# s3prl/s3prl

Hardware: AMD Instinct MI355X
Metric: encoder-frames/sec (20 ms stride) HuBERT-base 32x10 s @16 kHz (higher is better)
Workload: dtype f32; 1 GPU; hubert_base random-init, 32x10 s @16 kHz per GPU, one UpstreamExpert.forward per step: all 13 hidden_states (fp32) written; utterances_per_gpu=32, global_batch=32, samples=160000, frames_per_utt=499, parallelism=dp1, lengths=equal, gather=none

## Files before the change

include/s3enc.h:

```cpp
#ifndef S3ENC_H
#define S3ENC_H

#include <stdint.h>

#ifdef __cplusplus
extern "C" {
#endif

#define S3ENC_VERSION 8
#define S3ENC_MAX_CONV 16
#define S3ENC_MAX_RES 4

typedef struct s3enc_encoder* s3enc_handle;

enum { S3ENC_HUBERT = 0, S3ENC_WAV2VEC2 = 1, S3ENC_WAVLM = 2,
       S3ENC_DISTILLER = 3,
       S3ENC_MULTIRES = 4,
       S3ENC_WAV2VEC = 5,
       S3ENC_CPC = 6,
       S3ENC_APC = 7,
       S3ENC_MOCKINGJAY = 8,
       S3ENC_DECOAR = 9,
       S3ENC_NPC = 10 };
enum { S3ENC_F32 = 0, S3ENC_BF16 = 1, S3ENC_F16 = 2,
// ... 203 lines not shown
                               int64_t recv_state_stride, int32_t n_states, int64_t bytes_per_state, void* const* ready_events,
                               void* stream);
int s3enc_comm_destroy(s3enc_comm c);

int s3enc_forward_padded(s3enc_handle h, const float* pcm, int64_t row_stride, const int64_t* lengths, int32_t B,
                         int64_t n_max, float* out, int64_t layer_stride, void* stream);

int s3enc_profile_enable(s3enc_handle h, int32_t on);
int s3enc_profile_reset(s3enc_handle h);
typedef struct s3enc_profile_entry {
    char name[48];
    int64_t launches;
    double ms;
    double flops;
    double bytes;
} s3enc_profile_entry;
int s3enc_profile_read(s3enc_handle h, s3enc_profile_entry* entries, int32_t max_entries, int32_t* n_entries);

int s3enc_debug_tap(s3enc_handle h, const char* name, float* host_out, int64_t max_elems, int64_t* n_elems);
int s3enc_debug_occupy_cus(int32_t workgroups, int32_t threads, double milliseconds, void* stream);
int s3enc_debug_clock_sample(uint64_t* out3_device, void* stream);
int s3enc_debug_gemm_schedule(int32_t M, int32_t N, int32_t batches, int32_t tm, int32_t tail, int32_t cus, int32_t* items4_host,
                              int64_t max_items, int64_t* n_items);

int s3enc_set_tuning(const char* key, int32_t value);
int s3enc_set_handle_tuning(s3enc_handle h, const char* key, int32_t value);


int s3enc_op_gemm(int32_t dtype, const void* A, int64_t lda, int64_t a_batch_stride, const void* W,
                  const float* bias, int32_t M, int32_t N, int32_t K, int32_t batches, int32_t act,
                  const float* residual, const int32_t* row_limit, float* out32, void* out16, int64_t ldo,
                  int64_t o_batch_stride, void* stream);

int s3enc_op_conv0(int32_t dtype, const float* const* wavs, const int64_t* lengths, int32_t B, int64_t n_max,
                   int32_t normalize, const float* w0, const float* bias, const float* gn_gamma, const float* gn_beta,
                   const float* ln_gamma, const float* ln_beta, int32_t C, int32_t stride, void* out, void* stream);
int s3enc_op_wavlm_gate(const float* x, const float* grep_w, const float* grep_b, const float* grep_a, int32_t B, int32_t T,
                        int32_t H, float* gate, void* stream);

int s3enc_op_layernorm(int32_t dtype, const float* x, const float* gamma, const float* beta, int32_t rows,
                       int32_t C, int32_t act, float* out32, void* out16, void* stream);

int s3enc_op_attention(int32_t dtype, const void* qkv, void* out, const int32_t* valid, int32_t B, int32_t T,
                       int32_t H, const float* bias_table, int32_t table_R, const float* gate, void* stream);

int s3enc_op_conformer_conv(const float* x, const float* taps, const float* shift, int32_t B, int32_t T, int32_t D, int32_t K,
                            float* out, void* stream);
int s3enc_op_relpos_attention(const float* qkv, float* out, const int32_t* valid, int32_t B, int32_t T, int32_t H, const float* P,
                              const float* qadd, void* stream);

int s3enc_op_gn1_apply(const float* x, const float* gamma, const float* beta, const float* res, float scale, int32_t log_compress,
                       int32_t B, int32_t rows, int32_t C, int32_t pad, int32_t pad_zero, float* dst, float* state, float* acc,
                       float acc_w, int32_t acc_norm, int32_t acc_init, void* stream);
int s3enc_op_argmax_gather(const float* scores, const float* table, int32_t shared, int64_t rows, int32_t G, int32_t V, int32_t Dv,
                           int64_t* ids, float* out, void* stream);

int s3enc_op_channelnorm_relu(const float* x, const float* gamma, const float* beta, int32_t B, int32_t rows, int32_t C,
                              int32_t pad, float* dst, float* state, void* stream);
int s3enc_op_rnn(int32_t cell, const float* pre, const float* w_hh_host, const float* b_hn, int32_t B, int32_t T, int32_t H,
                 int64_t ld_pre, float* out, int64_t ldo, void* stream);

int s3enc_op_rnn_len(int32_t cell, const float* pre, const float* w_hh_host, const float* b_hn, const int32_t* len_host,
                     const float* res, int64_t ld_res, int32_t B, int32_t T, int32_t H, int64_t ld_pre, float* out, int64_t ldo,
                     void* stream);

int s3enc_op_conv_taps(const float* x, const float* w_host, const float* bias, int32_t B, int32_t T, int32_t C, int32_t N, int32_t k,
// ... 48 lines not shown
```

s3prl_amd/_lib.py:

```python

from __future__ import annotations

import ctypes as C
import os

_HERE = os.path.dirname(os.path.abspath(__file__))
LIB_PATH = os.path.join(_HERE, "libs3enc.so")

S3ENC_MAX_CONV = 16
S3ENC_MAX_RES = 4
F32, BF16, F16, F32X3, F16X2 = 0, 1, 2, 3, 4
STATUS_NONFINITE, STATUS_PENDING = 1, 1 << 30
DTYPES = {"fp32": F32, "f32": F32, "float32": F32, "bf16": BF16, "bfloat16": BF16, "fp16": F16, "f16": F16,
          "float16": F16, "fp32x3": F32X3, "f32x3": F32X3, "bf16x3": F32X3,
          "fp16x2": F16X2, "f16x2": F16X2}
FAMILY = {"hubert": 0, "wav2vec2": 1, "wavlm": 2, "distiller": 3, "multires_hubert": 4, "wav2vec": 5, "cpc": 6, "apc": 7, "mockingjay": 8, "decoar": 9, "npc": 10}
CPC_NORM = {"layerNorm": 0, "instanceNorm": 1, "ID": 2, "batchNorm": 3}
CPC_AR = {"LSTM": 0, "GRU": 1, "RNN": 2, "transformer": 3, "no_ar": 4}
APC_WINDOW = {"povey": 0, "hamming": 1}
VQ_TYPE = {"none": 0, "gumbel": 1, "kmeans": 2}
SEL_HIDDEN, SEL_LAYER_OUT, SEL_FFN_OUT = 0, 1, 2
SELECTIONS = {None: SEL_HIDDEN, "hidden_states": SEL_HIDDEN, "fairseq_layers": SEL_LAYER_OUT,
              "fairseq_layers_before_residual": SEL_FFN_OUT}
ABI_VERSION = 8
# ... 103 lines not shown
    "s3enc_create_npc": (C.c_int, [C.POINTER(S3Config), C.POINTER(S3NpcConfig), C.POINTER(S3Tensor), _I32, _I32, C.POINTER(_VP)]),
    "s3enc_destroy": (C.c_int, [_VP]),
    "s3enc_num_frames": (C.c_int, [_VP, _I64, C.POINTER(_I32)]),
    "s3enc_num_output_frames": (C.c_int, [_VP, _I64, C.POINTER(_I32)]),
    "s3enc_downsample_rate": (C.c_int, [_VP, C.POINTER(_I32)]),
    "s3enc_valid_frames": (C.c_int, [_VP, _I64, _I64, C.POINTER(_I32)]),
    "s3enc_forward": (C.c_int, [_VP, C.POINTER(_VP), C.POINTER(_I64), _I32, _I64, _VP, _I64, _VP]),
    "s3enc_forward_status": (C.c_int, [_VP, _I32, C.POINTER(_I32)]),
    "s3enc_forward_ex": (C.c_int, [_VP, C.POINTER(_VP), C.POINTER(_I64), _I32, _I64, C.POINTER(S3ForwardOpts), _VP, _I64, _VP]),
    "s3enc_forward_aux": (C.c_int, [_VP, C.POINTER(_VP), C.POINTER(_I64), _I32, _I64, C.POINTER(S3ForwardOpts), _VP, _I64, _VP, _VP, _VP]),
    "s3enc_num_states": (C.c_int, [_VP, _I32, C.POINTER(_I32)]),
    "s3enc_forward_padded": (C.c_int, [_VP, _VP, _I64, C.POINTER(_I64), _I32, _I64, _VP, _I64, _VP]),
    "s3enc_set_layer_events": (C.c_int, [_VP, C.POINTER(_VP), _I32]),
    "s3enc_profile_enable": (C.c_int, [_VP, _I32]),
    "s3enc_profile_reset": (C.c_int, [_VP]),
    "s3enc_profile_read": (C.c_int, [_VP, C.POINTER(S3ProfileEntry), _I32, C.POINTER(_I32)]),
    "s3enc_debug_tap": (C.c_int, [_VP, C.c_char_p, C.POINTER(C.c_float), _I64, C.POINTER(_I64)]),
    "s3enc_comm_version": (C.c_int, [C.POINTER(_I32)]),
    "s3enc_comm_unique_id": (C.c_int, [_VP]),
    "s3enc_comm_init_rank": (C.c_int, [_VP, _I32, _I32, _I32, C.POINTER(_VP)]),
    "s3enc_comm_info": (C.c_int, [_VP, C.POINTER(_I32), C.POINTER(_I32)]),
    "s3enc_comm_allgather_states": (C.c_int, [_VP, _VP, _I64, _VP, _I64, _I32, _I64, C.POINTER(_VP), _VP]),
    "s3enc_comm_exchange_states": (C.c_int, [_VP, _I32, _VP, _I64, _VP, _I64, _I32, _I64, C.POINTER(_VP), _VP]),
    "s3enc_comm_destroy": (C.c_int, [_VP]),
    "s3enc_comm_init_local": (C.c_int, [_I32, _I32, _I32, C.POINTER(_VP)]),
    "s3enc_comm_copy_export": (C.c_int, [_VP, _VP, _I64, _VP]),
    "s3enc_comm_copy_attach": (C.c_int, [_VP, _VP]),
    "s3enc_comm_copy_status": (C.c_int, [_VP, C.POINTER(_I32)]),
    "s3enc_comm_copy_release": (C.c_int, [_VP, _VP]),
    "s3enc_set_handle_tuning": (C.c_int, [_VP, C.c_char_p, _I32]),
    "s3enc_set_tuning": (C.c_int, [C.c_char_p, _I32]),
    "s3enc_op_gemm": (C.c_int, [_I32, _VP, _I64, _I64, _VP, _VP, _I32, _I32, _I32, _I32, _I32, _VP, _VP, _VP, _VP,
                                _I64, _I64, _VP]),
    "s3enc_debug_occupy_cus": (C.c_int, [_I32, _I32, C.c_double, _VP]),
    "s3enc_debug_clock_sample": (C.c_int, [_VP, _VP]),
    "s3enc_debug_gemm_schedule": (C.c_int, [_I32, _I32, _I32, _I32, _I32, _I32, _VP, _I64, C.POINTER(_I64)]),
    "s3enc_op_layernorm": (C.c_int, [_I32, _VP, _VP, _VP, _I32, _I32, _I32, _VP, _VP, _VP]),
    "s3enc_op_attention": (C.c_int, [_I32, _VP, _VP, _VP, _I32, _I32, _I32, _VP, _I32, _VP, _VP]),
    "s3enc_op_conv0": (C.c_int, [_I32, C.POINTER(_VP), C.POINTER(_I64), _I32, _I64, _I32, _VP, _VP, _VP, _VP, _VP, _VP, _I32,
                                 _I32, _VP, _VP]),
    "s3enc_op_wavlm_gate": (C.c_int, [_VP, _VP, _VP, _VP, _I32, _I32, _I32, _VP, _VP]),
    "s3enc_op_conformer_conv": (C.c_int, [_VP, _VP, _VP, _I32, _I32, _I32, _I32, _VP, _VP]),
    "s3enc_op_gn1_apply": (C.c_int, [_VP, _VP, _VP, _VP, C.c_float, _I32, _I32, _I32, _I32, _I32, _I32, _VP, _VP, _VP, C.c_float,
                                     _I32, _I32, _VP]),
    "s3enc_op_channelnorm_relu": (C.c_int, [_VP, _VP, _VP, _I32, _I32, _I32, _I32, _VP, _VP, _VP]),
    "s3enc_op_rnn": (C.c_int, [_I32, _VP, _VP, _VP, _I32, _I32, _I32, _I64, _VP, _I64, _VP]),
    "s3enc_op_rnn_len": (C.c_int, [_I32, _VP, _VP, _VP, _VP, _VP, _I64, _I32, _I32, _I32, _I64, _VP, _I64, _VP]),
    "s3enc_op_lstm_bidir": (C.c_int, [_VP, _VP, _VP, _VP, _VP, _I32, _I32, _I32, _I64, _VP, _I64, _VP]),
    "s3enc_pack_lstm_bidir_whh": (C.c_int, [_VP, _I32, _VP]),
    "s3enc_op_conv_taps": (C.c_int, [_VP, _VP, _VP, _I32, _I32, _I32, _I32, _I32, _I32, _I32, _VP, _I64, _VP, _I32, _I64, _VP, _VP,
                                     _I32, _I32, _VP]),
    "s3enc_op_argmax_gather": (C.c_int, [_VP, _VP, _I32, _I64, _I32, _I32, _I32, _VP, _VP, _VP]),
    "s3enc_op_relpos_attention": (C.c_int, [_VP, _VP, _VP, _I32, _I32, _I32, _VP, _VP, _VP]),
    "s3enc_op_posconv": (C.c_int, [_I32, _VP, _VP, _VP, _I32, _I32, _I32, _I32, _I32, _VP, _VP]),
    "s3enc_weighted_sum": (C.c_int, [_VP, _I64, _I32, C.POINTER(C.c_float), _I32, _I64, _I32, _VP, _VP]),
    "s3enc_weighted_sum_backward_scratch": (_I64, [_I64, _I32]),
    "s3enc_weighted_sum_backward": (C.c_int, [_VP, _I64, _I32, _I32, _I64, _I32, _VP, _VP, _VP, _VP]),
    "s3enc_fbank_num_frames": (C.c_int, [C.POINTER(S3FbankConfig), _I64, C.POINTER(_I32)]),
    "s3enc_fbank_forward": (C.c_int, [C.POINTER(S3FbankConfig), _VP, C.POINTER(_I64), _I32, _VP, _I64, _I32, _VP]),
    "s3enc_fbank_forward_ex": (C.c_int, [C.POINTER(S3FbankConfig), _I32, _VP, C.POINTER(_I64), _I32, _VP, _I64, _I32, _VP]),
    "s3enc_logmel_frame_counts": (C.c_int, [C.POINTER(_I64), _I32, _I64, C.POINTER(_I32)]),
    "s3enc_logmel_forward": (C.c_int, [_VP, C.POINTER(_I64), _I32, _I64, _I32, C.c_float, _I32, C.POINTER(_I32), _VP, _I32, _VP]),
    "s3enc_op_layernorm_eps": (C.c_int, [_VP, _VP, _VP, C.c_float, _I64, _I32, _VP, _VP]),
    "s3enc_op_input_repr": (C.c_int, [_VP, _VP, _VP, _VP, _I32, _VP, _VP, C.c_float, _I64, _I32, _I32, _VP, _VP]),
}

# ... 187 lines not shown
```

s3prl_amd/csrc/engine.hip:

```cpp
#include "engine_internal.h"

namespace s3e {

thread_local std::string g_err;

long conv_len(const s3enc_config& c, long n, int upto ) {
    for (int i = 0; i < upto; ++i) n = n >= c.conv_kernel[i] ? (n - c.conv_kernel[i]) / c.conv_stride[i] + 1 : 0;
    return n;
}

int valid_frames(const s3enc_config& c, long length, long n_max) {
    const long T = conv_len(c, n_max, c.n_conv);
    if (T <= 0) return 0;
    long v;
    if (c.family == S3ENC_WAV2VEC2 || c.family == S3ENC_DISTILLER || c.family == S3ENC_WAV2VEC || c.family == S3ENC_APC || c.family == S3ENC_NPC) {
        v = conv_len(c, length, c.n_conv);
    } else {
        const long chunk = n_max / T;
        v = (length + chunk - 1) / chunk;
    }
    if (v > T) v = T;
    if (v < 0) v = 0;
    return (int)v;
}
// ... 328 lines not shown
            std::unique_ptr<MxImage> img(new MxImage());              \
            UP(upload_mx4_lo(*img, vec, N_, K_));                     \
            img->kind = KIND;                                         \
            e->mx_images[(buf).p] = std::move(img);                   \
        }                                                             \
    } while (0)

    if (e->x2 && !c.no_feature_layer_norm && c.n_conv >= 3) {
        bool ok = true;
        for (int i = 2; i < c.n_conv; ++i) ok = ok && x3_shape_ok(C, (long)c.conv_kernel[i] * C, (long)c.conv_stride[i] * C);
        if (ok) e->x2_conv_f32_from = 2;
        if (ok && tuning().fp16x2_conv1_f32 && x3_shape_ok(C, (long)c.conv_kernel[1] * C, (long)c.conv_stride[1] * C)) e->x2_conv_f32_from = 1;
    }
    e->conv.resize(c.n_conv);
    for (int i = 0; i < c.n_conv; ++i) {
        const std::string p = "feature_extractor.conv_layers." + std::to_string(i);
        const int cin = i == 0 ? 1 : C, k = c.conv_kernel[i];
        GET(p + ".0.weight", (long)C * cin * k, t);
        if (i == 0) {
            UP(upload_f32(e->conv[i].w, t));
        } else {
            tap_major(t, C, cin, k, t2);
            if (e->x2_conv_f32_from && i >= e->x2_conv_f32_from) {
                UP(upload_gemm_w(e->conv[i].w, t2, C, (long)k * cin, e->dtype, e->x2));
            } else {
                UPW(e->conv[i].w, t2, C, (long)k * cin, 1);
            }
            if (e->x3 || (e->x2_conv_f32_from && i >= e->x2_conv_f32_from)) UP(upload_x3(e->conv[i].w3, t2, C, (long)k * cin));
            if (e->dtype == F32 && !e->x3 && k == 3 && c.conv_stride[i] == 2) {
                std::vector<float> wp((size_t)C * cin);
                for (int co = 0; co < C; ++co)
                    for (int ci = 0; ci < cin; ++ci) wp[(size_t)co * cin + ci] = t2[(long)co * 3 * cin + ci] + t2[(long)co * 3 * cin + 2 * cin + ci];
                UP(upload_f32(e->conv[i].wp, wp));
            }
        }
        if (c.conv_bias) {
            GET(p + ".0.bias", C, t);
            UP(upload_f32(e->conv[i].bias, t));
            e->conv[i].has_bias = true;
        }
        if (c.extractor_layer_norm) {
            GET(p + ".2.1.weight", C, t);
            UP(upload_f32(e->conv[i].lng, t));
            GET(p + ".2.1.bias", C, t);
            UP(upload_f32(e->conv[i].lnb, t));
        } else if (i == 0) {
            GET(p + ".2.weight", C, t);
            UP(upload_f32(e->gn_g, t));
            GET(p + ".2.bias", C, t);
            UP(upload_f32(e->gn_b, t));
        }
    }
    if (!c.no_feature_layer_norm) {
        GET("layer_norm.weight", C, t);
        UP(upload_f32(e->fln_g, t));
        GET("layer_norm.bias", C, t);
        UP(upload_f32(e->fln_b, t));
    }
    GET("post_extract_proj.weight", (long)D * C, t);
    UP(upload_gemm_w(e->proj_w, t, D, C, e->dtype, e->x2));
    e->x2_proj_f32 = e->x2 && !c.no_feature_layer_norm && c.family != S3ENC_DISTILLER && x3_shape_ok(D, C, C);
    if (e->x3 || e->x2_proj_f32) UP(upload_x3(e->proj_w3, t, D, C));
    GET("post_extract_proj.bias", D, t);
    UP(upload_f32(e->proj_b, t));

    const bool conf = c.layer_type == 1;
// ... 630 lines not shown
    if (T < 1) return fail("s3enc_forward: input shorter than the receptive field of the conv stack");
    const long M = (long)B * T;
    MrPlan plan;
    if (mr) mr_plan(c, T, plan);
    for (const auto& bp : plan.blocks)
        if (bp.T < 1 || plan.T_out < 1) return fail("s3enc_forward: input too short for the coarsest resolution of the U-net");
    const long out_rows = mr ? (long)B * plan.T_out : M;
    if (check_out(out, fo, layer_stride, out_rows * D)) return 1;
    if (c.rel_pos && T > 6000) return fail("s3enc_forward: WavLM relative-position window limited to 6000 frames (120 s) per batch");
    if (conf && T > 100000) return fail("s3enc_forward: Conformer position tables are limited to 100000 frames (max_source_positions)");
    std::vector<int> valid(B);
    for (int b = 0; b < B; ++b) {
        valid[b] = valid_frames(c, lengths[b], n_max);
        if (valid[b] < 1) return fail("s3enc_forward: an utterance is too short to produce a valid frame");
    }
    std::vector<int> valid_blk;
    if (mr) {
        std::vector<int> v = valid;
        for (size_t bi = 1; bi < plan.blocks.size(); ++bi) {
            const MrBlockPlan& bp = plan.blocks[bi];
            const AdapterW& aw = e->mr_adapters[bp.adapter];
            const long up = aw.kind == 1 ? 1 : aw.up_rate, down = aw.kind == 2 ? 1 : aw.down_rate;
            for (int b = 0; b < B; ++b) {
                long nv = ((long)v[b] * up + down - 1) / down;
                v[b] = (int)std::min(nv, bp.T);
            }
            valid_blk.insert(valid_blk.end(), v.begin(), v.end());
            for (int b = 0; b < B; ++b) v[b] = (int)std::min<long>(v[b], bp.T_sum);
        }
    }
    DeviceGuard dg(e->device);
    if (!dg.ok) return fail("s3enc_forward: hipSetDevice failed");

    const size_t tbl_bytes = (size_t)B * (8 + 8 + 4) + valid_blk.size() * 4;
    const size_t part_elems = stats_partial_elems(B, n_max);
    {
        Bump sb(nullptr);
        sb.take(tbl_bytes);
        sb.take((size_t)B * sizeof(float2));
        sb.take((size_t)B * C * sizeof(float2));
        sb.take(part_elems * 8);
        HIP_TRY(e->small.ensure_on_stream(sb.off + 1024, st));
    }
    Bump sb(e->small.p);
    char* d_tbl = (char*)sb.take(tbl_bytes);
    float2* d_norm = (float2*)sb.take((size_t)B * sizeof(float2));
    float2* d_gn = (float2*)sb.take((size_t)B * C * sizeof(float2));
    double* d_part = (double*)sb.take(part_elems * 8);
    const float* const* d_ptrs = (const float* const*)d_tbl;
    const long* d_lens = (const long*)(d_tbl + (size_t)B * 8);
    const int* d_valid = (const int*)(d_tbl + (size_t)B * 16);

    char* hp;
    if (stage_begin(e, tbl_bytes, st, hp)) return 1;
    memcpy(hp, wav_ptrs_host, (size_t)B * 8);
    for (int b = 0; b < B; ++b) ((long*)(hp + (size_t)B * 8))[b] = (long)lengths[b];
    memcpy(hp + (size_t)B * 16, valid.data(), (size_t)B * 4);
    if (!valid_blk.empty()) memcpy(hp + (size_t)B * 20, valid_blk.data(), valid_blk.size() * 4);
    if (stage_commit(e, hp, d_tbl, tbl_bytes, st)) return 1;

    const bool lnmode = c.extractor_layer_norm != 0;
    const bool prel = c.layer_norm_first != 0;
    const bool gated = c.rel_pos && c.gru_rel_pos;
    const bool featln = !c.no_feature_layer_norm;
    const bool ffn_tap = fo.selection == S3ENC_SEL_FFN_OUT;
    const long HW = std::max<long>(F, (long)NH * D);
    void *actA, *actB, *tmp32, *feat32, *featT, *x32, *xpc, *xT, *qkv, *attn, *tmp1, *tmp2, *hbuf, *gate, *ffnbuf, *lnst, *cbuf, *pbuf;
    for (int pass = 0; pass < 2; ++pass) {
        Bump wb(pass ? e->ws.p : nullptr);
        actA = wb.take(std::max((size_t)B * L[0] * C * (e->x2_conv_f32_from == 1 ? 4 : es),
                                (e->x2_conv_f32_from && c.n_conv > 2) ? (size_t)B * L[2] * C * 4 : (size_t)0));
        actB = wb.take((size_t)B * L[1] * C * (e->x2_conv_f32_from ? 4 : es));
        tmp32 = lnmode ? wb.take((size_t)B * L[1] * C * 4) : nullptr;
        feat32 = featln ? wb.take((size_t)M * C * 4) : nullptr;
        featT = wb.take((size_t)M * C * (e->x2_proj_f32 ? 4 : es));
        x32 = wb.take((size_t)M * D * 4);
        xpc = wb.take((size_t)M * D * 4);
        xT = wb.take((size_t)M * D * es);
        qkv = wb.take((size_t)M * 3 * D * es);
        attn = wb.take((size_t)M * D * (e->x2_attn_f32 ? 4 : es));
        tmp1 = wb.take((size_t)M * D * 4);
        tmp2 = wb.take((size_t)M * D * 4);
        lnst = wb.take((size_t)M * sizeof(float2));
        hbuf = wb.take((size_t)M * HW * es);
        gate = gated ? wb.take((size_t)B * H * T * 4) : nullptr;
        ffnbuf = (ffn_tap && (fo.featurize || fo.out_dtype != F32)) ? wb.take((size_t)M * D * 4) : nullptr;
        cbuf = conf ? wb.take((size_t)M * 2 * D * 4) : nullptr;
        pbuf = (conf && c.pos_enc_type == 1) ? wb.take((size_t)(2 * T - 1) * D * 4) : nullptr;
        if (!pass) HIP_TRY(e->ws.ensure_on_stream(wb.off + 4096, st));
        static const int dbg_poison = getenv("S3ENC_DEBUG_POISON") ? atoi(getenv("S3ENC_DEBUG_POISON")) : 0;
        if (pass && dbg_poison) HIP_TRY(hipMemsetAsync(e->ws.p, 0xFF, wb.off, st));
// ... 77 lines not shown
        GemmParams g{};
        g.A = cur;
        g.lda = (long)c.conv_stride[i] * C;
        g.a_bs = L[i - 1] * C;
        g.W = e->conv[i].w.p;
        g.W_x3 = e->conv[i].w3.p;
        g.bias = e->conv[i].has_bias ? (const float*)e->conv[i].bias.p : nullptr;
        g.M = (int)L[i];
        g.N = C;
        g.K = c.conv_kernel[i] * C;
        g.batches = B;
        g.ldo = C;
        g.o_bs = L[i] * C;
        const double fl = 2.0 * B * L[i] * C * g.K;
        const double by = ((double)B * L[i - 1] * C + (double)C * g.K) * (x3in ? 4 : es) + (double)B * L[i] * C * (f32out ? 4 : es);
        char kind[32];
        snprintf(kind, sizeof(kind), "gemm:conv%d", i);
        ConvF22Params f22{};
        bool use_f22 = false;
        if (dt == F32 && !e->x3 && !x3in && c.conv_kernel[i] == 3 && c.conv_stride[i] == 2 && e->conv[i].wp.p) {
            f22.x = (const float*)cur;
            f22.x_bs = L[i - 1] * C;
            f22.W = (const float*)e->conv[i].w.p;
            f22.WP = (const float*)e->conv[i].wp.p;
            f22.bias = g.bias;
            f22.M = (int)L[i];
            f22.C = C;
            f22.batches = B;
            f22.act = lnmode ? 0 : 1;
            f22.out = (float*)(lnmode ? tmp32 : dst);
            f22.o_bs = L[i] * C;
            use_f22 = conv_f22_eligible(f22);
        }
        if (!lnmode) {
            g.act = 1;
            if (f32out) g.out32 = (float*)dst; else g.out16 = dst;
            Prof pr(e, st, kind, fl, by);
            if (use_f22) {
                HIP_TRY(launch_conv_f22(f22, st));
            } else if (x3in) {
                if (!gemm_x3_eligible(g)) return fail("conv layer is not a shape of the three-term GEMM (internal)");
                HIP_TRY(launch_gemm(F32, g, st));
            } else {
                HIP_TRY(launch_gemm(dt, wsplit_of(e, g), st));
            }
        } else {
            g.act = 0;
            g.out32 = (float*)tmp32;
            {
                Prof pr(e, st, kind, fl, by);
                if (use_f22) {
                    HIP_TRY(launch_conv_f22(f22, st));
                } else if (x3in) {
                    if (!gemm_x3_eligible(g)) return fail("conv layer is not a shape of the three-term GEMM (internal)");
                    HIP_TRY(launch_gemm(F32, g, st));
                } else {
                    HIP_TRY(launch_gemm(dt, wsplit_of(e, g), st));
                }
            }
            Prof pr(e, st, "layernorm:conv", 0, (double)B * L[i] * C * (4 + (f32out ? 4 : es)));
            HIP_TRY(launch_layernorm(dt, (const float*)tmp32, (const float*)e->conv[i].lng.p, (const float*)e->conv[i].lnb.p,
                                     (long)B * L[i], C, e->x3 ? 2 : 1, f32out ? (float*)dst : nullptr, f32out ? nullptr : dst, st));
        }
        char tn[16];
        snprintf(tn, sizeof(tn), "conv%d", i);
        if (i >= c.n_conv - 3 || dbg_stop) e->taps[tn] = {dst, (long)B * L[i] * C, f32out ? (int)F32 : dt};
        else HIP_TRY(keep_tap(tn, i, dst, (long)B * L[i] * C, f32out ? (int)F32 : dt));
        if (dbg_stop == 1 + i) return 0;
        cur = dst;
    }
    const bool proj32 = dt == F32 || (e->x2_proj_f32 && featln);
    if (featln) {
        Prof pr(e, st, "layernorm:feat", 0, (double)M * C * (4 + (proj32 ? 4 : es)));
        HIP_TRY(launch_layernorm(dt, (const float*)feat32, (const float*)e->fln_g.p, (const float*)e->fln_b.p, M, C, 0,
                                 proj32 ? (float*)featT : nullptr, proj32 ? nullptr : featT, st));
        e->taps["feat_ln"] = {featT, M * C, proj32 ? (int)F32 : dt};
        if (dbg_stop == 20) return 0;
    }
    const int si_proj = (dist || (conf && c.layer_norm_first)) ? 0 : -1;
    float* xproj = sink.slot32(si_proj) ? sink.slot32(si_proj) : (float*)x32;
    {
        GemmParams g{};
        g.A = featT;
        g.lda = C;
// ... 528 lines not shown
```

s3prl_amd/csrc/engine_internal.h:

```cpp
#pragma once
#include <hip/hip_runtime.h>

#include <algorithm>
#include <cmath>
#include <cstdio>
#include <cstring>
#include <map>
#include <memory>
#include <mutex>
#include <string>
#include <thread>
#include <vector>

#include "../../include/s3enc.h"
#include "kernels.h"

namespace s3e {
using namespace s3;


extern thread_local std::string g_err;

inline int fail(const std::string& msg) {
    g_err = msg;
// ... 262 lines not shown
    return hipMemcpy(d.p, pk.data(), pk.size() * 2, hipMemcpyHostToDevice);
}

inline hipError_t upload_posconv_x3(DevBuf& d, const std::vector<float>& w, int D, int G, int K) {
    std::vector<float> lay;
    pack_posconv(w, D, G, K, BF16, lay);
    std::vector<uint16_t> img(lay.size() * 2);
    for (size_t i = 0; i < lay.size(); ++i) {
        const uint16_t h = h_bf16(lay[i]);
        img[i] = h;
        img[lay.size() + i] = h_bf16(lay[i] - h_from16(h, BF16));
    }
    hipError_t e = d.ensure(img.size() * 2 + 16);
    if (e != hipSuccess) return e;
    return hipMemcpy(d.p, img.data(), img.size() * 2, hipMemcpyHostToDevice);
}

struct LayerW {
    DevBuf wqkv, bqkv, wo, bo, ln1g, ln1b, w1, b1, w2, b2, ln2g, ln2b;
    DevBuf wqkv3, wo3, w13, w23;
    DevBuf grep_w, grep_b, grep_a;
};
struct ConformerLayerW {
    DevBuf f1_lng, f1_lnb, f1_w1, f1_b1, f1_w2, f1_b2;
    DevBuf at_lng, at_lnb, wqkv, bqkv, wo, bo, wpos, qadd;
    DevBuf cv_lng, cv_lnb, pw1, taps, shift, pw2;
    DevBuf f2_lng, f2_lnb, f2_w1, f2_b1, f2_w2, f2_b2;
    DevBuf fin_g, fin_b;
};
struct ConvW {
    DevBuf w, bias, lng, lnb;
    DevBuf w3;
    DevBuf wp;
    bool has_bias = false;
};

struct BlockW {
    std::vector<LayerW> layers;
    DevBuf eln_g, eln_b;
};
struct AdapterConvW {
    DevBuf w, w3;
    DevBuf g, b;
};
struct AdapterW {
    AdapterConvW up, down;
    int kind = 0;
    int up_rate = 1, down_rate = 1;
};

struct W2vW {
    std::vector<DevBuf> ext_w, ext_g, ext_b;
    std::vector<DevBuf> agg_w, agg_bias, agg_g, agg_b;
    std::vector<DevBuf> vq_w, vq_b;
    std::vector<DevBuf> km_w;
    DevBuf km_g, km_b, emb_t;
    DevBuf table;
};

struct RnnW {
    std::vector<DevBuf> w_ih, b_pre, w_hh, b_hn;
};
int load_rnn_layer(const Ckpt& ck, const std::string& prefix, const std::string& suffix, int G, int H, int I, RnnW& w);

struct CpcW : RnnW {
    std::vector<DevBuf> conv_w, conv_b, cn_g, cn_b;
// ... 348 lines not shown
```

s3prl_amd/csrc/kernels.h:

```cpp
#pragma once
#include <cstring>
#include <vector>

#include "common.h"

namespace s3 {
int device_cus();

template <auto Kern>
inline hipError_t ensure_dynamic_lds(int bytes) {
    static int granted[64] = {};
    int dev = 0;
    hipError_t e = hipGetDevice(&dev);
    if (e != hipSuccess) return e;
    if (dev >= 0 && dev < 64 && granted[dev] >= bytes) return hipSuccess;
    e = hipFuncSetAttribute((const void*)Kern, hipFuncAttributeMaxDynamicSharedMemorySize, bytes);
    if (e == hipSuccess && dev >= 0 && dev < 64) granted[dev] = bytes;
    return e;
}

struct Tuning {
    int gemm_variant = 3;
    int gemm_lds_pad = 0;
    int gemm32_big = 1;
    int gemm_x3_tile = 1;
    int gemm32_tail = 1;
    int gemm32_tail_units = 0;
    int gemm16_big = 3;
    int gemm16_pp = 0;
    int gemm16_mx = 14;
    int reserve_cus = 0;
    int gemm16_rows = 1;
    int attn_lds_pad = 0;
    int attn_persist = 0;
    int conv0_nt = 1;
    int conv_f22 = 1;
    int conv0_fast = 1;
    int ws_inplace = 1;
    int gelu32 = 1;
    int x3_pack_cache = 0;
    int fp16x2_conv1_f32 = 0;
    int ln_rows = 1;
    int ln_preload = 1;
    int ln1_fold = 1;
    int gn_lag_one_block = 1;
    int forward_chain = 1;
    int rnn_split = -1;
    int npc_skip_taps = 1;
    int comm_self_p2p = 0;
};
extern Tuning g_tuning;
extern thread_local const Tuning* t_tuning;
inline const Tuning& tuning() { return t_tuning ? *t_tuning : g_tuning; }
struct TuningScope {
    const Tuning* prev;
    explicit TuningScope(const Tuning* t) : prev(t_tuning) { if (t) t_tuning = t; }
    ~TuningScope() { t_tuning = prev; }
};
int tuning_set(Tuning& t, const char* key, int value, const char** err);

extern thread_local int* t_status;
struct StatusScope {
    int* prev;
    explicit StatusScope(int* p) : prev(t_status) { t_status = p; }
    ~StatusScope() { t_status = prev; }
};

struct GemmParams {
    const void* A;
// ... 18 lines not shown
    const void* W4s = nullptr;
    int mxw = 0;
};
bool gemm16_mx_eligible(int dtype, const GemmParams& p);
bool gemm16_mx_weight_rule(long N, long K);
bool gemm_x3_eligible(const GemmParams& p);
hipError_t launch_gemm_x3(const GemmParams& p, hipStream_t stream);
void pack_x3(const float* w, long N, long K, std::vector<uint16_t>& out);
bool gemm16_big_eligible(int dtype, const GemmParams& p);
bool gemm16_res_ln_ok(int dtype, const GemmParams& p);
hipError_t launch_gemm16_big(int dtype, const GemmParams& p, hipStream_t stream);
bool gemm_tile_eligible(int dtype, const GemmParams& p);
struct GemmTileSched {
    int tm, m_bulk, m_tail;
};
GemmTileSched gemm_tile_schedule(int M, int N, int batches, int tm, int tail_mode, int tail_units, int cus);
void gemm_tile_items(int M, int N, int batches, const GemmTileSched& s, std::vector<int>& items4);
hipError_t launch_gemm_tile(int dtype, const GemmParams& p, hipStream_t stream);
hipError_t launch_gemm(int dtype, const GemmParams& p, hipStream_t stream);
struct ConvF22Params {
    const float* x;
    long x_bs;
    const float* W;
    const float* WP;
    const float* bias;
    int M, C, batches;
    int act;
    const int* row_limit;
    float* out;
    long o_bs;
};
bool conv_f22_eligible(const ConvF22Params& p);
hipError_t launch_conv_f22(const ConvF22Params& p, hipStream_t stream);
struct ConvTapsParams {
    const float* src;
    long src_bs;
    int C;
    const float* W;
    const float* bias;
    int T, N, B;
    int taps0, gap, taps1;
    int act;
    const float* res;
    long res_bs, ld_res;
    float* dst;
    long dst_bs, ld_dst;
    float* state;
    long state_bs, ld_state;
    float* sum;
    long sum_bs, ld_sum;
    int sum_init;
};
void pack_conv_taps(const float* w, int N, int C, int k, int mask, bool dense, std::vector<float>& out);
const char* conv_taps_refusal(const ConvTapsParams& p);
hipError_t launch_conv_taps(const ConvTapsParams& p, hipStream_t stream);

struct WavTable {
    const float* const* ptrs;
    const long* lens;
    int B;
    long n_max;
};
constexpr int STAT_K0_MAX = 16;
hipError_t launch_wav_norm_stats(const WavTable& w, int normalize, double* partial, float2* norm, hipStream_t s,
                                 float eps = 0.f );
hipError_t launch_gn_stats(const WavTable& w, const float2* norm, const float* w0 , const float* gamma,
// ... 293 lines not shown
```

s3prl_amd/csrc/ops.hip:

```cpp
#include "engine_internal.h"

namespace s3 {
Tuning g_tuning;
thread_local const Tuning* t_tuning = nullptr;
thread_local int* t_status = nullptr;

int tuning_set(Tuning& t, const char* key, int value, const char** err) {
    struct Key {
        const char* name;
        int Tuning::*field;
        int lo, hi;
    };
    static const Key keys[] = {
        {"gemm_variant", &Tuning::gemm_variant, 0, 63},      {"gemm_lds_pad", &Tuning::gemm_lds_pad, 0, 120 * 1024},
        {"gemm32_big", &Tuning::gemm32_big, 0, 5},           {"gemm_x3_tile", &Tuning::gemm_x3_tile, 0, 5},
        {"gemm16_big", &Tuning::gemm16_big, 0, 10},          {"gemm16_rows", &Tuning::gemm16_rows, 0, 1},
        {"attn_lds_pad", &Tuning::attn_lds_pad, 0, 48 * 1024}, {"conv0_nt", &Tuning::conv0_nt, 0, 1},
        {"ws_inplace", &Tuning::ws_inplace, 0, 1},           {"gemm16_pp", &Tuning::gemm16_pp, 0, 3},
        {"gemm16_mx", &Tuning::gemm16_mx, 0, 31},            {"reserve_cus", &Tuning::reserve_cus, 0, 128},
        {"x3_pack_cache", &Tuning::x3_pack_cache, 0, 1},     {"gelu32", &Tuning::gelu32, 0, 1},
        {"comm_self_p2p", &Tuning::comm_self_p2p, 0, 1},     {"attn_persist", &Tuning::attn_persist, 0, 1},
        {"fp16x2_conv1_f32", &Tuning::fp16x2_conv1_f32, 0, 1}, {"gn_lag_one_block", &Tuning::gn_lag_one_block, 0, 1},
        {"ln_rows", &Tuning::ln_rows, 1, 2},                 {"ln1_fold", &Tuning::ln1_fold, 0, 1},
        {"ln_preload", &Tuning::ln_preload, 0, 1},           {"forward_chain", &Tuning::forward_chain, 0, 1},
        {"conv0_fast", &Tuning::conv0_fast, 0, 1},           {"conv_f22", &Tuning::conv_f22, 0, 1},
        {"rnn_split", &Tuning::rnn_split, -1, 8},           {"npc_skip_taps", &Tuning::npc_skip_taps, 0, 1},
        {"gemm32_tail", &Tuning::gemm32_tail, 0, 2},         {"gemm32_tail_units", &Tuning::gemm32_tail_units, 0, 1 << 20},
    };
    static thread_local char msg[160];
    if (!key) {
        *err = "s3enc_set_tuning: null key";
        return 1;
    }
    for (const Key& k : keys)
        if (!strcmp(key, k.name)) {
            if (value < k.lo || value > k.hi) {
                snprintf(msg, sizeof(msg), "%s must be %d..%d", k.name, k.lo, k.hi);
                *err = msg;
                return 1;
            }
            t.*(k.field) = value;
            return 0;
        }
    snprintf(msg, sizeof(msg), "s3enc_set_tuning: unknown key '%s'", key);
    *err = msg;
    return 1;
}
}

extern "C" {

int s3enc_set_tuning(const char* key, int32_t value) {
    const char* err = nullptr;
    if (tuning_set(g_tuning, key, value, &err)) return fail(err);
    return 0;
}
int s3enc_set_handle_tuning(s3enc_handle h, const char* key, int32_t value) {
    if (!h) return fail("null handle");
    if (!h->has_tuning) {
        h->tun = g_tuning;
        h->has_tuning = true;
    }
    const char* err = nullptr;
    if (tuning_set(h->tun, key, value, &err)) return fail(err);
    return 0;
}

int s3enc_op_gemm(int32_t dtype, const void* A, int64_t lda, int64_t a_batch_stride, const void* W, const float* bias, int32_t M,
                  int32_t N, int32_t K, int32_t batches, int32_t act, const float* residual, const int32_t* row_limit,
                  float* out32, void* out16, int64_t ldo, int64_t o_batch_stride, void* stream) {
    GemmParams g{};
    g.A = A;
    g.lda = lda;
    g.a_bs = a_batch_stride;
    g.W = W;
    g.bias = bias;
    g.M = M;
    g.N = N;
    g.K = K;
    g.batches = batches;
    g.act = act;
    g.residual = residual;
    g.row_limit = row_limit;
    g.out32 = out32;
    g.out16 = out16;
    g.ldo = ldo;
    g.o_bs = o_batch_stride;
    if (dtype == 4) {
        g.wsplit = 1;
        HIP_TRY(launch_gemm(F16, g, (hipStream_t)stream));
        return 0;
    }
    if (dtype == 5) {
        std::vector<float> hw((size_t)N * K);
        HIP_TRY(hipMemcpy(hw.data(), W, hw.size() * 4, hipMemcpyDeviceToHost));
        DevBuf w2;
        MxImage img;
        HIP_TRY(upload_gemm_w(w2, hw, N, K, F16, true));
        HIP_TRY(upload_mx4_lo(img, hw, N, K));
        g.W = w2.p;
// ... 711 lines not shown
```

Measured before the change: 461,300 frames/s.

## Add three-output fast-convolution kernel for k3 s2 feature-extractor conv layers

Result: no change. 464,700 frames/s (median of 6 runs) (+0.7%).

```diff
diff --git a/include/s3enc.h b/include/s3enc.h
--- a/include/s3enc.h
+++ b/include/s3enc.h
@@ -259,6 +259,10 @@
                   const float* residual, const int32_t* row_limit, float* out32, void* out16, int64_t ldo,
                   int64_t o_batch_stride, void* stream);
 
+int s3enc_op_conv_k3s2(int32_t form, const float* x, int64_t x_batch_stride, const float* W, const float* aux0, const float* aux1,
+                       const float* bias, int32_t M, int32_t C, int32_t batches, int32_t act, const int32_t* row_limit,
+                       const int32_t* own_rows, float* out, int64_t o_batch_stride, void* stream);
+
 int s3enc_op_conv0(int32_t dtype, const float* const* wavs, const int64_t* lengths, int32_t B, int64_t n_max,
                    int32_t normalize, const float* w0, const float* bias, const float* gn_gamma, const float* gn_beta,
                    const float* ln_gamma, const float* ln_beta, int32_t C, int32_t stride, void* out, void* stream);
diff --git a/s3prl_amd/_lib.py b/s3prl_amd/_lib.py
--- a/s3prl_amd/_lib.py
+++ b/s3prl_amd/_lib.py
@@ -159,6 +159,7 @@
     "s3enc_set_tuning": (C.c_int, [C.c_char_p, _I32]),
     "s3enc_op_gemm": (C.c_int, [_I32, _VP, _I64, _I64, _VP, _VP, _I32, _I32, _I32, _I32, _I32, _VP, _VP, _VP, _VP,
                                 _I64, _I64, _VP]),
+    "s3enc_op_conv_k3s2": (C.c_int, [_I32, _VP, _I64, _VP, _VP, _VP, _VP, _I32, _I32, _I32, _I32, _VP, _VP, _VP, _I64, _VP]),
     "s3enc_debug_occupy_cus": (C.c_int, [_I32, _I32, C.c_double, _VP]),
     "s3enc_debug_clock_sample": (C.c_int, [_VP, _VP]),
     "s3enc_debug_gemm_schedule": (C.c_int, [_I32, _I32, _I32, _I32, _I32, _I32, _VP, _I64, C.POINTER(_I64)]),
diff --git a/s3prl_amd/csrc/convf3x2.hip b/s3prl_amd/csrc/convf3x2.hip
--- /dev/null
+++ b/s3prl_amd/csrc/convf3x2.hip
@@ -0,0 +1,289 @@
+#include <type_traits>
+
+#include "kernels.h"
+
+namespace s3 {
+
+namespace {
+
+constexpr int TR = 64, BM = 3 * TR, ROWB = 64;
+static_assert(BM == CONV_F3X2_TILE_ROWS, "tile height");
+typedef int i32x4 __attribute__((ext_vector_type(4)));
+
+__device__ __forceinline__ uint4 sub4(const uint4& a, const uint4& b) {
+    return make_uint4(__float_as_uint(__uint_as_float(a.x) - __uint_as_float(b.x)), __float_as_uint(__uint_as_float(a.y) - __uint_as_float(b.y)),
+                      __float_as_uint(__uint_as_float(a.z) - __uint_as_float(b.z)), __float_as_uint(__uint_as_float(a.w) - __uint_as_float(b.w)));
+}
+__device__ __forceinline__ uint4 add4(const uint4& a, const uint4& b) {
+    return make_uint4(__float_as_uint(__uint_as_float(a.x) + __uint_as_float(b.x)), __float_as_uint(__uint_as_float(a.y) + __uint_as_float(b.y)),
+                      __float_as_uint(__uint_as_float(a.z) + __uint_as_float(b.z)), __float_as_uint(__uint_as_float(a.w) + __uint_as_float(b.w)));
+}
+__device__ __forceinline__ void mma4(const uint4& a, const uint4& b, f32x16& c) {
+    c = __builtin_amdgcn_mfma_f32_32x32x2f32(__uint_as_float(a.x), __uint_as_float(b.x), c, 0, 0, 0);
+    c = __builtin_amdgcn_mfma_f32_32x32x2f32(__uint_as_float(a.y), __uint_as_float(b.y), c, 0, 0, 0);
+    c = __builtin_amdgcn_mfma_f32_32x32x2f32(__uint_as_float(a.z), __uint_as_float(b.z), c, 0, 0, 0);
+    c = __builtin_amdgcn_mfma_f32_32x32x2f32(__uint_as_float(a.w), __uint_as_float(b.w), c, 0, 0, 0);
+}
+
+template <int NJ>
+struct Lay {
+    static constexpr int BN = 64 * NJ;
+    static constexpr int A_W1 = 192;
+    static constexpr int B_E1 = 64, B_E2 = 128, B_W0 = 192, B_W2 = 192 + BN, B_E064 = 192 + 2 * BN;
+    static constexpr int C_E2 = 64, C_GP = 128, C_GM = 128 + BN;
+    static constexpr int ROWS = B_E064 + 16;
+    static constexpr int PLANE = ROWS * ROWB;
+    static constexpr int NF = 4 + 2 * NJ;
+};
+
+template <int NJ>
+__global__ __launch_bounds__(256, NJ == 2 ? 2 : 3) void conv_f3x2_kernel(ConvF3x2Params p) {
+    using L = Lay<NJ>;
+    constexpr int BN = L::BN, PLANE = L::PLANE;
+    extern __shared__ __attribute__((aligned(16))) char smem[];
+    const int tid = threadIdx.x;
+    const int lane = tid & 63;
+    const int wave = __builtin_amdgcn_readfirstlane(tid >> 6);
+    const int pb = wave >> 1, wc = wave & 1;
+    const int half = lane >> 5;
+    const int l31 = lane & 31;
+    const int C = p.C, N = p.C;
+
+    int tile;
+    {
+        const int nwg = gridDim.x, wg = blockIdx.x;
+        const int q8 = nwg >> 3, r8 = nwg & 7, xcd = wg & 7, loc = wg >> 3;
+        tile = (xcd < r8 ? xcd * (q8 + 1) : r8 * (q8 + 1) + (xcd - r8) * q8) + loc;
+    }
+    const int n_tiles = (N + BN - 1) / BN;
+    const int m_tiles = (p.M + 2 + BM - 1) / BM;
+    const int tn = tile % n_tiles;
+    const int tmb = tile / n_tiles;
+    const int tm = tmb % m_tiles, b = tmb / m_tiles;
+    const int own = p.own_rows ? p.own_rows[b] : p.M;
+    const int base = own % 3 > 0 ? own % 3 - 3 : 0;
+    const int m0 = base + tm * BM, n0 = tn * BN;
+    if (m0 >= p.M) return;
+    const int nc = C >> 4;
+
+    i32x4 rsrc_x, rsrc_w, rsrc_p, rsrc_m;
+    {
+        const unsigned long ux = (unsigned long)(p.x + (long)b * p.x_bs), uw = (unsigned long)p.W, up = (unsigned long)p.GP, um = (unsigned long)p.GM;
+        rsrc_x = (i32x4){(int)__builtin_amdgcn_readfirstlane((unsigned)ux), (int)__builtin_amdgcn_readfirstlane((unsigned)(ux >> 32)), -1, 0x00020000};
+        rsrc_w = (i32x4){(int)__builtin_amdgcn_readfirstlane((unsigned)uw), (int)__builtin_amdgcn_readfirstlane((unsigned)(uw >> 32)), -1, 0x00020000};
+        rsrc_p = (i32x4){(int)__builtin_amdgcn_readfirstlane((unsigned)up), (int)__builtin_amdgcn_readfirstlane((unsigned)(up >> 32)), -1, 0x00020000};
+        rsrc_m = (i32x4){(int)__builtin_amdgcn_readfirstlane((unsigned)um), (int)__builtin_amdgcn_readfirstlane((unsigned)(um >> 32)), -1, 0x00020000};
+    }
+    const unsigned sl16 = (unsigned)(((lane & 3) ^ ((lane >> 4) & 3)) << 4);
+    const int fmax = 2 * p.M;
+    const int rl = 16 * wave + (lane >> 2);
+    const int fb = 2 * base + 6 * (tm * TR + rl);
+    const int fb64 = 2 * base + 6 * (tm * TR + TR + (lane >> 2));
+    int wn[NJ];
+#pragma unroll
+    for (int j = 0; j < NJ; ++j) wn[j] = min(n0 + rl + 64 * j, N - 1);
+    const unsigned lds0 = __builtin_amdgcn_readfirstlane((unsigned)(uintptr_t)(__attribute__((address_space(3))) char*)smem) + wave * 1024;
+    auto dma = [&](unsigned vo, const i32x4& rs, unsigned dst, unsigned soff) {
+        asm volatile("s_mov_b32 m0, %0\n\ts_nop 0\n\tbuffer_load_dwordx4 %1, %2, %3 offen lds"
+                     :
+                     : "s"(dst), "v"(vo), "s"(rs), "s"(soff)
+                     : "memory");
+    };
+    auto issue = [&](int ph, int kc, int slot) {
+        const unsigned d0 = lds0 + slot * PLANE;
+        int f = fb, f64 = fb64;
+        asm volatile("" : "+v"(f), "+v"(f64));
+        auto xoff = [&](int fr) { return (unsigned)min(max(fr, 0), fmax) * (unsigned)(C * 4) + sl16; };
+        const unsigned kb = (unsigned)kc * ROWB;
+        if (ph == 0) {
+#pragma unroll
+            for (int i = 0; i < 3; ++i) dma(xoff(f + 1 + 2 * i), rsrc_x, d0 + i * 4096, kb);
+#pragma unroll
+            for (int j = 0; j < NJ; ++j) dma((unsigned)wn[j] * (unsigned)(3 * C * 4) + sl16, rsrc_w, d0 + (3 + j) * 4096, kb + (unsigned)(C * 4));
+        } else if (ph == 1) {
+#pragma unroll
+            for (int i = 0; i < 3; ++i) dma(xoff(f + 2 * i), rsrc_x, d0 + i * 4096, kb);
+#pragma unroll
+            for (int j = 0; j < NJ; ++j) {
+                const unsigned wo = (unsigned)wn[j] * (unsigned)(3 * C * 4) + sl16;
+                dma(wo, rsrc_w, d0 + (3 + j) * 4096, kb);
+                dma(wo, rsrc_w, d0 + (3 + NJ + j) * 4096, kb + (unsigned)(2 * C * 4));
+            }
+            if (wave == 0) dma(xoff(f64), rsrc_x, d0 + (3 + 2 * NJ) * 4096, kb);
+        } else {
+#pragma unroll
+            for (int i = 0; i < 2; ++i) dma(xoff(f + 2 + 2 * i), rsrc_x, d0 + i * 4096, kb);
+#pragma unroll
+            for (int j = 0; j < NJ; ++j) {
+                const unsigned go = (unsigned)wn[j] * (unsigned)(C * 4) + sl16;
+                dma(go, rsrc_p, d0 + (2 + j) * 4096, kb);
+                dma(go, rsrc_m, d0 + (2 + NJ + j) * 4096, kb);
+            }
+        }
+    };
+
+    auto rowoff = [&](int row) { return row * ROWB + (((half * 2) ^ ((row >> 2) & 3)) << 4); };
+    const int a_off = rowoff(pb * 32 + l31);
+    const int a1_off = rowoff(pb * 32 + l31 + 1 < TR ? pb * 32 + l31 + 1 : L::B_E064);
+    const int w_off = rowoff(wc * 32 * NJ + l31);
+
+    f32x16 acc_y[3][NJ], acc_s[NJ], acc_d[NJ];
+#pragma unroll
+    for (int j = 0; j < NJ; ++j)
+#pragma unroll
+        for (int r = 0; r < 16; ++r) acc_y[0][j][r] = acc_y[1][j][r] = acc_y[2][j][r] = acc_s[j][r] = acc_d[j][r] = 0.f;
+
+    struct Frag {
+        uint4 v[L::NF];
+    };
+    auto read = [&](Frag& f, auto ph_c, int slot, int q) {
+        constexpr int ph = decltype(ph_c)::value;
+        const char* base = smem + slot * PLANE;
+        const int ao = a_off ^ (q << 4), a1o = a1_off ^ (q << 4), wo = w_off ^ (q << 4);
+        if constexpr (ph == 0) {
+#pragma unroll
+            for (int i = 0; i < 3; ++i) f.v[i] = *(const uint4*)(base + ao + i * 64 * ROWB);
+#pragma unroll
+            for (int j = 0; j < NJ; ++j) f.v[3 + j] = *(const uint4*)(base + wo + (L::A_W1 + j * 32) * ROWB);
+        } else if constexpr (ph == 1) {
+            f.v[0] = *(const uint4*)(base + ao);
+            f.v[1] = *(const uint4*)(base + a1o);
+            f.v[2] = *(const uint4*)(base + ao + L::B_E1 * ROWB);
+            f.v[3] = *(const uint4*)(base + ao + L::B_E2 * ROWB);
+#pragma unroll
+            for (int j = 0; j < NJ; ++j) {
+                f.v[4 + j] = *(const uint4*)(base + wo + (L::B_W0 + j * 32) * ROWB);
+                f.v[4 + NJ + j] = *(const uint4*)(base + wo + (L::B_W2 + j * 32) * ROWB);
+            }
+        } else {
+            f.v[0] = *(const uint4*)(base + ao);
+            f.v[1] = *(const uint4*)(base + ao + L::C_E2 * ROWB);
+#pragma unroll
+            for (int j = 0; j < NJ; ++j) {
+                f.v[2 + j] = *(const uint4*)(base + wo + (L::C_GP + j * 32) * ROWB);
+                f.v[2 + NJ + j] = *(const uint4*)(base + wo + (L::C_GM + j * 32) * ROWB);
+            }
+        }
+    };
+    auto mma = [&](const Frag& f, auto ph_c, int g) {
+        constexpr int ph = decltype(ph_c)::value;
+        if constexpr (ph == 0) {
+            mma4(f.v[g / NJ], f.v[3 + g % NJ], acc_y[g / NJ][g % NJ]);
+        } else if constexpr (ph == 1) {
+            if (g < NJ) mma4(sub4(f.v[0], f.v[3]), f.v[4 + g], acc_y[0][g]);
+            else mma4(sub4(f.v[1], f.v[2]), f.v[4 + g], acc_y[2][g - NJ]);
+        } else {
+            if (g < NJ) mma4(add4(f.v[0], f.v[1]), f.v[2 + g], acc_s[g]);
+            else mma4(sub4(f.v[1], f.v[0]), f.v[2 + g], acc_d[g - NJ]);
+        }
+    };
+
+    const std::integral_constant<int, 0> PA{};
+    const std::integral_constant<int, 1> PB{};
+    const std::integral_constant<int, 2> PC{};
+    issue(0, 0, 0);
+    asm volatile("s_waitcnt vmcnt(0)" ::: "memory");
+    __builtin_amdgcn_s_barrier();
+    asm volatile("" ::: "memory");
+    issue(1, 0, 1);
+    Frag f0, f1;
+    read(f0, PA, 0, 0);
+    const int ns = 3 * nc;
+    auto step = [&](int s, int slot, auto ph_c, auto next_c, int iph, int ikc) {
+        constexpr int ng = decltype(ph_c)::value == 0 ? 3 * NJ : 2 * NJ;
+        read(f1, ph_c, slot, 1);
+#pragma unroll
+        for (int g = 0; g < ng; ++g) mma(f0, ph_c, g);
+        __builtin_amdgcn_sched_barrier(0);
+        asm volatile("s_waitcnt vmcnt(0) lgkmcnt(0)" ::: "memory");
+        __builtin_amdgcn_s_barrier();
+        asm volatile("" ::: "memory");
+        __builtin_amdgcn_sched_barrier(0);
+        mma(f1, ph_c, 0);
+        __builtin_amdgcn_sched_barrier(0);
+        if (s + 2 < ns) issue(iph, ikc, slot);
+        if (s + 1 < ns) read(f0, next_c, slot ^ 1, 0);
+        __builtin_amdgcn_sched_barrier(0);
+#pragma unroll
+        for (int g = 1; g < ng; ++g) mma(f1, ph_c, g);
+    };
+    for (int s = 0, c = 0; s < ns; s += 6, c += 2) {
+        step(s, 0, PA, PB, 2, c);
+        step(s + 1, 1, PB, PC, 0, c + 1);
+        step(s + 2, 0, PC, PA, 1, c + 1);
+        step(s + 3, 1, PA, PB, 2, c + 1);
+        step(s + 4, 0, PB, PC, 0, c + 2);
+        step(s + 5, 1, PC, PA, 1, c + 2);
+    }
+
+    const int limit = p.row_limit ? p.row_limit[b] : p.M;
+    const long ob = (long)b * p.o_bs;
+    constexpr int WN = 32 * NJ, LPR = WN / 4, RPP = 64 / LPR;
+    float* stg = (float*)(smem + wave * (32 * WN * 4));
+    const int c4 = (lane % LPR) * 4;
+    const int n = n0 + wc * WN + c4;
+    const bool n_ok = n < N;
+    float4 bias4 = make_float4(0.f, 0.f, 0.f, 0.f);
+    if (p.bias && n_ok) bias4 = *(const float4*)(p.bias + n);
+#pragma unroll
+    for (int q = 0; q < 3; ++q) {
+#pragma unroll
+        for (int j = 0; j < NJ; ++j)
+#pragma unroll
+            for (int r = 0; r < 16; ++r) {
+                const float sd = q == 1 ? acc_s[j][r] - acc_d[j][r] : acc_s[j][r] + acc_d[j][r];
+                stg[((r & 3) + 8 * (r >> 2) + 4 * half) * WN + j * 32 + l31] = acc_y[q][j][r] + sd;
+            }
+        asm volatile("s_waitcnt lgkmcnt(0)" ::: "memory");
+#pragma unroll
+        for (int t = 0; t < 32 / RPP; ++t) {
+            const int row = t * RPP + lane / LPR;
+            float4 v = *(const float4*)(stg + row * WN + c4);
+            const int m = m0 + 3 * (pb * 32 + row) + q;
+            if (m >= 0 && m < p.M && n_ok) {
+                v.x += bias4.x; v.y += bias4.y; v.z += bias4.z; v.w += bias4.w;
+                if (p.act == 2) {
+                    gelu_fast4(v);
+                } else if (p.act) {
+                    v.x = gelu_erf(v.x); v.y = gelu_erf(v.y); v.z = gelu_erf(v.z); v.w = gelu_erf(v.w);
+                }
+                if (m >= limit) v = make_float4(0.f, 0.f, 0.f, 0.f);
+                *(float4*)(p.out + ob + (long)m * C + n) = v;
+            }
+        }
+        asm volatile("s_waitcnt lgkmcnt(0)" ::: "memory");
+    }
+}
+
+template <int NJ>
+hipError_t launch(const ConvF3x2Params& p, hipStream_t stream) {
+    constexpr int lds = 2 * Lay<NJ>::PLANE, BN = Lay<NJ>::BN;
+    static_assert(lds >= 4 * 32 * 32 * NJ * 4, "the epilogue stages in the planes");
+    hipError_t e = ensure_dynamic_lds<conv_f3x2_kernel<NJ>>(lds);
+    if (e != hipSuccess) return e;
+    dim3 grid(((p.M + 2 + BM - 1) / BM) * ((p.C + BN - 1) / BN) * p.batches);
+    hipLaunchKernelGGL(conv_f3x2_kernel<NJ>, grid, dim3(256), lds, stream, p);
+    return hipGetLastError();
+}
+
+}
+
+bool conv_f3x2_eligible(const ConvF3x2Params& p) {
+    if (!tuning().conv_f3x2 || !p.x || !p.W || !p.GP || !p.GM || !p.out) return false;
+    if (p.C < 32 || (p.C & 31) || (p.x_bs & 3) || (p.o_bs & 3)) return false;
+    const uintptr_t al = (uintptr_t)p.x | (uintptr_t)p.W | (uintptr_t)p.GP | (uintptr_t)p.GM | (uintptr_t)p.out | (uintptr_t)p.bias;
+    if (al & 15) return false;
+    const unsigned long x_span = ((unsigned long)p.x_bs + (unsigned long)p.C) * 4ul;
+    const unsigned long w_span = (unsigned long)p.C * 3ul * (unsigned long)p.C * 4ul;
+    return x_span < (1ul << 32) - 64 && w_span < (1ul << 32) - 64;
+}
+
+hipError_t launch_conv_f3x2(const ConvF3x2Params& p0, hipStream_t stream) {
+    ConvF3x2Params p = p0;
+    if (p.M <= 0 || p.batches <= 0) return hipSuccess;
+    if (!conv_f3x2_eligible(p) || (2L * p.M + 1) * p.C > p.x_bs) return hipErrorInvalidValue;
+    if (p.act == 1 && tuning().gelu32 == 1) p.act = 2;
+    return tuning().conv_f3x2 == 2 ? launch<1>(p, stream) : launch<2>(p, stream);
+}
+
+}
diff --git a/s3prl_amd/csrc/engine.hip b/s3prl_amd/csrc/engine.hip
--- a/s3prl_amd/csrc/engine.hip
+++ b/s3prl_amd/csrc/engine.hip
@@ -384,6 +384,15 @@
                 for (int co = 0; co < C; ++co)
                     for (int ci = 0; ci < cin; ++ci) wp[(size_t)co * cin + ci] = t2[(long)co * 3 * cin + ci] + t2[(long)co * 3 * cin + 2 * cin + ci];
                 UP(upload_f32(e->conv[i].wp, wp));
+                std::vector<float> gm((size_t)C * cin);
+                for (int co = 0; co < C; ++co)
+                    for (int ci = 0; ci < cin; ++ci) {
+                        const float w0 = t2[(long)co * 3 * cin + ci], w2 = t2[(long)co * 3 * cin + 2 * cin + ci];
+                        wp[(size_t)co * cin + ci] = (w0 + w2) * 0.5f;
+                        gm[(size_t)co * cin + ci] = (w0 - w2) * 0.5f;
+                    }
+                UP(upload_f32(e->conv[i].gp, wp));
+                UP(upload_f32(e->conv[i].gm, gm));
             }
         }
         if (c.conv_bias) {
@@ -1080,7 +1089,8 @@
     DeviceGuard dg(e->device);
     if (!dg.ok) return fail("s3enc_forward: hipSetDevice failed");
 
-    const size_t tbl_bytes = (size_t)B * (8 + 8 + 4) + valid_blk.size() * 4;
+    const size_t own_off = (size_t)B * (8 + 8 + 4) + valid_blk.size() * 4;
+    const size_t tbl_bytes = own_off + (size_t)c.n_conv * B * 4;
     const size_t part_elems = stats_partial_elems(B, n_max);
     {
         Bump sb(nullptr);
@@ -1098,6 +1108,7 @@
     const float* const* d_ptrs = (const float* const*)d_tbl;
     const long* d_lens = (const long*)(d_tbl + (size_t)B * 8);
     const int* d_valid = (const int*)(d_tbl + (size_t)B * 16);
+    const int* d_own_rows = (const int*)(d_tbl + own_off);
 
     char* hp;
     if (stage_begin(e, tbl_bytes, st, hp)) return 1;
@@ -1105,6 +1116,8 @@
     for (int b = 0; b < B; ++b) ((long*)(hp + (size_t)B * 8))[b] = (long)lengths[b];
     memcpy(hp + (size_t)B * 16, valid.data(), (size_t)B * 4);
     if (!valid_blk.empty()) memcpy(hp + (size_t)B * 20, valid_blk.data(), valid_blk.size() * 4);
+    for (int i = 0; i < c.n_conv; ++i)
+        for (int b = 0; b < B; ++b) ((int*)(hp + own_off))[(size_t)i * B + b] = (int)conv_len(c, lengths[b], i + 1);
     if (stage_commit(e, hp, d_tbl, tbl_bytes, st)) return 1;
 
     const bool lnmode = c.extractor_layer_norm != 0;
@@ -1248,11 +1261,31 @@
             f22.o_bs = L[i] * C;
             use_f22 = conv_f22_eligible(f22);
         }
+        ConvF3x2Params f3{};
+        bool use_f3 = false;
+        if (use_f22 && e->conv[i].gp.p && e->conv[i].gm.p) {
+            f3.x = f22.x;
+            f3.x_bs = f22.x_bs;
+            f3.W = f22.W;
+            f3.GP = (const float*)e->conv[i].gp.p;
+            f3.GM = (const float*)e->conv[i].gm.p;
+            f3.bias = f22.bias;
+            f3.M = f22.M;
+            f3.C = C;
+            f3.batches = B;
+            f3.act = f22.act;
+            f3.out = f22.out;
+            f3.o_bs = f22.o_bs;
+            f3.own_rows = d_own_rows + (size_t)i * B;
+            use_f3 = conv_f3x2_eligible(f3);
+        }
         if (!lnmode) {
             g.act = 1;
             if (f32out) g.out32 = (float*)dst; else g.out16 = dst;
             Prof pr(e, st, kind, fl, by);
-            if (use_f22) {
+            if (use_f3) {
+                HIP_TRY(launch_conv_f3x2(f3, st));
+            } else if (use_f22) {
                 HIP_TRY(launch_conv_f22(f22, st));
             } else if (x3in) {
                 if (!gemm_x3_eligible(g)) return fail("conv layer is not a shape of the three-term GEMM (internal)");
@@ -1265,7 +1298,9 @@
             g.out32 = (float*)tmp32;
             {
                 Prof pr(e, st, kind, fl, by);
-                if (use_f22) {
+                if (use_f3) {
+                    HIP_TRY(launch_conv_f3x2(f3, st));
+                } else if (use_f22) {
                     HIP_TRY(launch_conv_f22(f22, st));
                 } else if (x3in) {
                     if (!gemm_x3_eligible(g)) return fail("conv layer is not a shape of the three-term GEMM (internal)");
diff --git a/s3prl_amd/csrc/engine_internal.h b/s3prl_amd/csrc/engine_internal.h
--- a/s3prl_amd/csrc/engine_internal.h
+++ b/s3prl_amd/csrc/engine_internal.h
@@ -318,6 +318,7 @@
     DevBuf w, bias, lng, lnb;
     DevBuf w3;
     DevBuf wp;
+    DevBuf gp, gm;
     bool has_bias = false;
 };
 
diff --git a/s3prl_amd/csrc/kernels.h b/s3prl_amd/csrc/kernels.h
--- a/s3prl_amd/csrc/kernels.h
+++ b/s3prl_amd/csrc/kernels.h
@@ -35,6 +35,7 @@
     int attn_persist = 0;
     int conv0_nt = 1;
     int conv_f22 = 1;
+    int conv_f3x2 = 1;
     int conv0_fast = 1;
     int ws_inplace = 1;
     int gelu32 = 1;
@@ -119,6 +120,23 @@
 };
 bool conv_f22_eligible(const ConvF22Params& p);
 hipError_t launch_conv_f22(const ConvF22Params& p, hipStream_t stream);
+constexpr int CONV_F3X2_TILE_ROWS = 192;
+struct ConvF3x2Params {
+    const float* x;
+    long x_bs;
+    const float* W;
+    const float* GP;
+    const float* GM;
+    const float* bias;
+    int M, C, batches;
+    int act;
+    const int* row_limit;
+    const int* own_rows;
+    float* out;
+    long o_bs;
+};
+bool conv_f3x2_eligible(const ConvF3x2Params& p);
+hipError_t launch_conv_f3x2(const ConvF3x2Params& p, hipStream_t stream);
 struct ConvTapsParams {
     const float* src;
     long src_bs;
diff --git a/s3prl_amd/csrc/ops.hip b/s3prl_amd/csrc/ops.hip
--- a/s3prl_amd/csrc/ops.hip
+++ b/s3prl_amd/csrc/ops.hip
@@ -26,6 +26,7 @@
         {"conv0_fast", &Tuning::conv0_fast, 0, 1},           {"conv_f22", &Tuning::conv_f22, 0, 1},
         {"rnn_split", &Tuning::rnn_split, -1, 8},           {"npc_skip_taps", &Tuning::npc_skip_taps, 0, 1},
         {"gemm32_tail", &Tuning::gemm32_tail, 0, 2},         {"gemm32_tail_units", &Tuning::gemm32_tail_units, 0, 1 << 20},
+        {"conv_f3x2", &Tuning::conv_f3x2, 0, 2},
     };
     static thread_local char msg[160];
     if (!key) {
@@ -66,6 +67,27 @@
     return 0;
 }
 
+int s3enc_op_conv_k3s2(int32_t form, const float* x, int64_t x_batch_stride, const float* W, const float* aux0, const float* aux1,
+                       const float* bias, int32_t M, int32_t C, int32_t batches, int32_t act, const int32_t* row_limit,
+                       const int32_t* own_rows, float* out, int64_t o_batch_stride, void* stream) {
+    if (form == 2) {
+        ConvF22Params p{};
+        p.x = x; p.x_bs = x_batch_stride; p.W = W; p.WP = aux0; p.bias = bias;
+        p.M = M; p.C = C; p.batches = batches; p.act = act; p.row_limit = row_limit; p.out = out; p.o_bs = o_batch_stride;
+        if (!conv_f22_eligible(p)) return fail("s3enc_op_conv_k3s2: not a shape of the two-output kernel (C % 32, alignment, conv_f22 = 0)");
+        HIP_TRY(launch_conv_f22(p, (hipStream_t)stream));
+        return 0;
+    }
+    if (form == 3) {
+        ConvF3x2Params p{};
+        p.x = x; p.x_bs = x_batch_stride; p.W = W; p.GP = aux0; p.GM = aux1; p.bias = bias;
+        p.M = M; p.C = C; p.batches = batches; p.act = act; p.row_limit = row_limit; p.own_rows = own_rows; p.out = out; p.o_bs = o_batch_stride;
+        if (!conv_f3x2_eligible(p)) return fail("s3enc_op_conv_k3s2: not a shape of the three-output kernel (C % 32, alignment, conv_f3x2 = 0)");
+        HIP_TRY(launch_conv_f3x2(p, (hipStream_t)stream));
+        return 0;
+    }
+    return fail("s3enc_op_conv_k3s2: form must be 2 or 3");
+}
 int s3enc_op_gemm(int32_t dtype, const void* A, int64_t lda, int64_t a_batch_stride, const void* W, const float* bias, int32_t M,
                   int32_t N, int32_t K, int32_t batches, int32_t act, const float* residual, const int32_t* row_limit,
                   float* out32, void* out16, int64_t ldo, int64_t o_batch_stride, void* stream) {
```
